# Byshx/Poccala

Hardware: AMD Instinct MI355X
Metric: frames/sec GMM-score+fwd-bwd, 39-d MFCC, 2048-mix (higher is better)
Workload: dtype f32-class (f16x2 split operands, f32 accumulate; f64 dynamic programming)

## Files before the change

poccala_amd/csrc/gmm_score_split.hip:

```cpp
#include <stdlib.h>

#include "pcl_internal.h"

namespace {

#ifndef PCL_SPLIT_WG
#define PCL_SPLIT_WG 256
#endif
constexpr int WG = PCL_SPLIT_WG;
typedef float f16v __attribute__((ext_vector_type(16)));

#ifndef PCL_SPLIT16_NT
#define PCL_SPLIT16_NT 2
#endif
#ifndef PCL_SPLIT16_MINW
#define PCL_SPLIT16_MINW 3
#endif
#ifndef PCL_SPLIT16_MTS
#define PCL_SPLIT16_MTS 1
#endif
typedef _Float16 h8v __attribute__((ext_vector_type(8)));

template <int D, int NT>
__global__ __launch_bounds__(WG, PCL_SPLIT16_MINW * 256 / WG > 0 ? PCL_SPLIT16_MINW * 256 / WG : 1) void gmm_score_split16_kernel(
    const float *__restrict__ frames, const uint4 *__restrict__ pm, const float *__restrict__ fscale, const float *__restrict__ centers,
    int nmt_max, const ScoreTile *__restrict__ tiles, const ScoreSeg *__restrict__ segs, double *__restrict__ out,
    int *__restrict__ flags, const double *__restrict__ kzero, const int *__restrict__ n_on_pipe, const int *__restrict__ npt) {
    static_assert(D % 8 != 0, "the folded constants need a spare slot");
    constexpr int KS8 = (D + 7) / 8;
    constexpr int CH = 2 * KS8;
    constexpr int SC = D / 8, JC = D % 8;
    constexpr float FMAXH = 6.0e4f;
    const ScoreTile tile = tiles[blockIdx.x];
    const int lane = threadIdx.x & 63;
    const int wave = threadIdx.x >> 6;
    const int half = lane >> 5;
    const int col = lane & 31;
    if (tile.seg_lo >= tile.seg_hi) {
        if (threadIdx.x == 0) flags[blockIdx.x] = 0;
        return;
    }
    const int n_mtiles = npt[tile.state];
    __shared__ int s_ovf;
    if (threadIdx.x == 0) s_ovf = 0;
    __syncthreads();
    const int vend = segs[tile.seg_hi - 1].vstart + segs[tile.seg_hi - 1].len;
    const bool wave_active = tile.vstart + wave * NT * 32 < vend;
    if (n_mtiles == 0) {
        if (wave_active) {
            for (int c = 0; c < NT; ++c) {
                const int v = tile.vstart + (wave * NT + c) * 32 + col;
                if (v < vend && half == 0) {
                    int lo = tile.seg0;
                    const int hi = tile.seg_hi - 1;
                    while (lo < hi && segs[lo + 1].vstart <= v) ++lo;
                    const ScoreSeg sg = segs[lo];
                    out[sg.out0 + (long long)(v - sg.vstart) * sg.out_stride] = -INFINITY;
                }
            }
        }
        if (threadIdx.x == 0) flags[blockIdx.x] = 0;
        return;
    }

    h8v xb[NT][2][KS8];
    long long oidx[NT];
    bool valid[NT];
    const float *cen = centers + (size_t)tile.state * D;
    const float *fs = fscale + ((size_t)tile.state * 2 + half) * (KS8 * 8);
    bool ovf = false;
#pragma unroll
    for (int c = 0; c < NT; ++c) {
        int v = tile.vstart + (wave * NT + c) * 32 + col;
        valid[c] = v < vend;
        if (!valid[c]) v = tile.vstart;
        int lo = tile.seg0, hi = tile.seg_hi - 1;
        if (lo < hi && segs[lo + 1].vstart <= v) {
            ++lo;
            if (lo < hi && segs[lo + 1].vstart <= v) {
                ++lo;
                while (lo < hi) {
                    int mid = (lo + hi + 1) >> 1;
                    if (segs[mid].vstart <= v) lo = mid; else hi = mid - 1;
                }
            }
        }
        const ScoreSeg sg = segs[lo];
        const long long t = v - sg.vstart;
        const float *fp = frames + (sg.frame0 + t) * D;
#pragma unroll
        for (int s = 0; s < KS8; ++s)
#pragma unroll
            for (int j = 0; j < 8; ++j) {
                const int d = 8 * s + j;
                float val = 0.f;
                if (d < D) {
                    const float xc = fp[d] - cen[d];
                    val = (half ? xc : xc * xc) * fs[d];
                    ovf |= __builtin_fabsf(val) > FMAXH;
                    val = __builtin_fminf(__builtin_fmaxf(val, -FMAXH), FMAXH);
                }
                if (d == D) val = half ? 0.f : 1.f;
                const _Float16 h1 = (_Float16)val;
                xb[c][0][s][j] = h1;
                xb[c][1][s][j] = (_Float16)(val - (float)h1);
            }
        oidx[c] = sg.out0 + t * (long long)sg.out_stride;
    }
    if (__any(ovf) && lane == 0) s_ovf = 1;

    float sm[NT], ref[NT];
    bool inited[NT];
#pragma unroll
    for (int c = 0; c < NT; ++c) {
        sm[c] = 0.f;
        ref[c] = 0.f;
        inited[c] = false;
    }
    bool ref_ovf = false;

    constexpr int MTS = PCL_SPLIT16_MTS;
    __shared__ __attribute__((aligned(16))) uint4 abuf[2][MTS * CH * 64];
    const uint4 *pstate = pm + (size_t)tile.state * nmt_max * (CH * 64);
    const int wave_s = __builtin_amdgcn_readfirstlane(wave);
    auto dma = [&](int buf, int stage) {
        const uint4 *src = pstate + (size_t)stage * (MTS * CH * 64);
        const int nch = min(MTS, n_mtiles - stage * MTS) * CH;
        if constexpr (KS8 > 5) {
            for (int p = wave; p < nch; p += WG / 64)
                __builtin_amdgcn_global_load_lds((const __attribute__((address_space(1))) void *)(src + p * 64 + lane),
                                                 (__attribute__((address_space(3))) void *)&abuf[buf][p * 64], 16, 0, 0);
            return;
        }
#pragma unroll
        for (int i = 0; i < (MTS * CH + WG / 64 - 1) / (WG / 64); ++i) {
            const int p = wave_s + i * (WG / 64);
            if (p < nch)
                __builtin_amdgcn_global_load_lds((const __attribute__((address_space(1))) void *)(src + p * 64 + lane),
                                                 (__attribute__((address_space(3))) void *)&abuf[buf][p * 64], 16, 0, 0);
        }
    };

#ifdef PCL_SPLIT_STAMPS
    unsigned long long st_acc[4] = {0, 0, 0, 0}, st_t = 0;
#define SSTAMP(k) { const unsigned long long t_ = __builtin_amdgcn_s_memtime(); st_acc[k] += t_ - st_t; st_t = t_; }
#else
#define SSTAMP(k)
#endif
    auto process = [&](int mt) {
        const uint4 *ab = &abuf[(mt / MTS) & 1][(mt % MTS) * (CH * 64)];
        f16v acc[NT];
#pragma unroll
        for (int c = 0; c < NT; ++c)
#pragma unroll
            for (int r = 0; r < 16; ++r) acc[c][r] = 0.f;
        auto frag = [&](int pa, int s) { return *reinterpret_cast<const h8v *>(&ab[(pa * KS8 + s) * 64 + lane]); };
        auto mfma = [&](const h8v &a, int c, int pb, int s) { acc[c] = __builtin_amdgcn_mfma_f32_32x32x16_f16(a, xb[c][pb][s], acc[c], 0, 0, 0); };
        float es[8], eh, snew[NT];
        auto lse_op = [&](int c, int k) {
            if (k < 24) {
                const int r = k / 3;
                if (k % 3 == 0) es[r] = __builtin_amdgcn_exp2f(acc[c][r]);
                else if (k % 3 == 1) eh = __builtin_amdgcn_exp2f(acc[c][r + 8]);
                else es[r] += eh;
            } else if (k < 28) es[k - 24] += es[k - 24 + 4];
            else if (k < 30) es[k - 28] += es[k - 28 + 2];
            else if (k == 30) es[0] += es[1];
            else snew[c] = sm[c] + es[0];
        };
        if constexpr (KS8 <= 5) {
            h8v af[2 * KS8];
            auto rd = [&](int f) { af[f] = frag(f < KS8 ? 1 : 0, f % KS8); };
            constexpr int LATE = KS8 > 2 ? 2 : 0;
            rd(0);
            rd(1);
            __builtin_amdgcn_sched_barrier(0);
#ifdef PCL_SPLIT_PRIO
            __builtin_amdgcn_s_setprio(1);
#endif
#pragma unroll
            for (int s = 0; s < KS8; ++s) {
#pragma unroll
                for (int c = 0; c < NT; ++c) {
                    mfma(af[s], c, 0, s);
                    if (s == 0 && c == 0) {
                        __builtin_amdgcn_sched_barrier(0);
#pragma unroll
                        for (int f = 2; f < 2 * KS8 - LATE; ++f) rd(f);
                    }
                }
                if (s == 2) {
#pragma unroll
                    for (int f = 2 * KS8 - LATE; f < 2 * KS8; ++f) rd(f);
                }
                __builtin_amdgcn_sched_barrier(0);
            }
#pragma unroll
            for (int c = 0; c < NT; ++c) {
                int k = 0;
#pragma unroll
                for (int g = 0; g < 2 * KS8; ++g) {
                    mfma(af[KS8 + g % KS8], c, g < KS8 ? 1 : 0, g % KS8);
                    if (c == 0) __builtin_amdgcn_sched_barrier(0);
#ifndef PCL_DIAG_NOLSE
                    if (c > 0) {
#pragma unroll
                        for (int q = 0; q < 3 && k < 32; ++q, ++k) lse_op(c - 1, k);
                        __builtin_amdgcn_sched_barrier(0);
                    }
#endif
                }
#ifndef PCL_DIAG_NOLSE
                if (c > 0) {
#pragma unroll
                    for (; k < 32; ++k) lse_op(c - 1, k);
                }
#endif
                __builtin_amdgcn_sched_barrier(0);
            }
        } else {
            auto pass = [&](int pa, int pb) {
#pragma unroll
                for (int s = 0; s < KS8; ++s) {
                    const h8v a = frag(pa, s);
#pragma unroll
                    for (int c = 0; c < NT; ++c) mfma(a, c, pb, s);
                }
            };
            pass(1, 0);
            pass(0, 1);
            pass(0, 0);
#ifndef PCL_DIAG_NOLSE
#pragma unroll
            for (int c = 0; c + 1 < NT; ++c)
#pragma unroll
                for (int k = 0; k < 32; ++k) lse_op(c, k);
#endif
        }
#ifndef PCL_DIAG_NOLSE
#pragma unroll
        for (int k = 0; k < 32; ++k) lse_op(NT - 1, k);
#endif
        SSTAMP(1)
#ifdef PCL_SPLIT_PRIO
        __builtin_amdgcn_s_setprio(0);
#endif
#ifdef PCL_DIAG_NOLSE
#pragma unroll
        for (int c = 0; c < NT; ++c) sm[c] += acc[c][0] + acc[c][15];
        return;
#endif
#pragma unroll
        for (int c = 0; c < NT; ++c) {
            if (__any(!inited[c]) | __any(!(snew[c] < 3.0e38f))) {
                float gm = acc[c][0];
#pragma unroll
                for (int r = 1; r < 16; ++r) gm = __builtin_fmaxf(gm, acc[c][r]);
                const float gp = __builtin_fmaxf(gm, __shfl_xor(gm, 32, 64));
                float s = sm[c];
                const bool first = !inited[c];
                if ((first || gp > 0.f) && gp > -5.0e4f) {
                    const _Float16 r1 = (_Float16)__builtin_fminf(__builtin_fmaxf(-(ref[c] + gp), -FMAXH), FMAXH);
                    const float nref = -(float)r1, dl = nref - ref[c];
                    ref_ovf |= __builtin_fabsf(nref) > 5.0e4f;
#ifdef PCL_LSE_FLUSH_REPRO
                    s = first ? 0.f : s * __builtin_amdgcn_exp2f(-dl);
#else
                    const float hs = __builtin_amdgcn_exp2f(-0.5f * dl);
                    s = first ? 0.f : (s * hs) * hs;
#endif
                    inited[c] = true;
#pragma unroll
                    for (int r = 0; r < 16; ++r) acc[c][r] -= dl;
                    ref[c] = nref;
                    if (half) xb[c][0][SC][JC] = r1;
                }
#pragma unroll
                for (int r = 0; r < 16; ++r) s += __builtin_amdgcn_exp2f(acc[c][r]);
                sm[c] = s;
            } else {
                sm[c] = snew[c];
            }
        }
        SSTAMP(2)
    };
    const int n_stages = (n_mtiles + MTS - 1) / MTS;
    dma(0, 0);
#ifdef PCL_SPLIT_STAMPS
    st_t = __builtin_amdgcn_s_memtime();
#endif
    for (int st = 0; st < n_stages; ++st) {
        asm volatile("s_waitcnt vmcnt(0)" ::: "memory");
        SSTAMP(3)
        __syncthreads();
        SSTAMP(0)
        if (st == 0 && threadIdx.x == 0) flags[blockIdx.x] = s_ovf;
        if (st + 1 < n_stages) dma((st + 1) & 1, st + 1);
        if (wave_active) {
            const int mend = min(n_mtiles, (st + 1) * MTS);
            for (int mt = st * MTS; mt < mend; ++mt) process(mt);
        }
    }
#ifdef PCL_SPLIT_STAMPS
    if (blockIdx.x == 800 && lane == 0)
        printf("wave %d: per m-tile: dma-wait %llu  barrier %llu  dma-issue+lds+mfma %llu  lse %llu (memtime ticks)\n", wave,
               st_acc[3] / n_mtiles, st_acc[0] / n_mtiles, st_acc[1] / n_mtiles, st_acc[2] / n_mtiles);
#endif
    constexpr double LN2 = 0.693147180559945309417232121458;
    const double k0 = kzero[tile.state];
    if (wave_active && n_on_pipe[tile.state] > 0) {
#pragma unroll
        for (int c = 0; c < NT; ++c) ref_ovf |= !inited[c];
    }
#pragma unroll
    for (int c = 0; c < NT; ++c) {
        const double S = (double)sm[c] + (double)__shfl_xor(sm[c], 32, 64);
        if (valid[c] && half == 0) out[oidx[c]] = (S > 0) ? LN2 * ((double)ref[c] + k0 + ::log2(S)) : -INFINITY;
    }
    if (__any(ref_ovf) && lane == 0) s_ovf = 1;
    __syncthreads();
    if (threadIdx.x == 0 && s_ovf) flags[blockIdx.x] = 1;
}

template <int D>
void launch16_t(pcl_ctx *ctx, pcl_batch *b, const ScoreTile *tiles, int n_tiles) {
    constexpr size_t static_lds = 2 * (size_t)(2 * ((D + 7) / 8)) * 64 * 16;
    const size_t pad = (ctx->score_wgs_per_cu == 2 && static_lds < (56u << 10)) ? (56u << 10) - static_lds : 0;
    hipLaunchKernelGGL((gmm_score_split16_kernel<D, PCL_SPLIT16_NT>), dim3(n_tiles), dim3(WG), pad, ctx->stream, ctx->frames32,
                       reinterpret_cast<const uint4 *>(ctx->pm16f.p), ctx->fscale, ctx->centers32, ctx->Mpad32 / 32, tiles, b->d_segs,
                       b->Bt, b->d_tile_flags, ctx->kzero, ctx->d_non, ctx->d_npt);
}

}

int pcl_score_split16_tile_frames() { return WG / 64 * PCL_SPLIT16_NT * 32; }

int pcl_launch_score_split16(pcl_ctx *ctx, pcl_batch *b, const ScoreTile *tiles, int n_tiles) {
    if (n_tiles == 0) return PCL_OK;
    pcl_timer_begin(ctx, "score");
    switch (ctx->D) {
#define CASE(DD) case DD: launch16_t<DD>(ctx, b, tiles, n_tiles); break;
        PCL_MFMA_DIMS(CASE)
#undef CASE
        default: PCL_FAIL(ctx, PCL_ERR_INVALID, "internal: no split-f16 scoring kernel for D=%d", ctx->D);
    }
    pcl_timer_end(ctx, "score");
    HIPCHK(ctx, hipGetLastError());
    return PCL_OK;
}
```

Before: 21.64 million.

## Generalize LDS double buffer into configurable ring with partial vmcnt waits

Replaces the fixed two-buffer LDS prefetch of Gaussian parameter tiles with a templated ring of R stages. When R>2 it waits only on older loads via partial vmcnt counts and uses a raw barrier. It also raises the default number of m-tiles per stage from one to two, halving barriers per tile at the cost of more LDS per workgroup. Static asserts check that the ring still fits three workgroups per CU.

```diff
diff --git a/poccala_amd/csrc/gmm_score_split.hip b/poccala_amd/csrc/gmm_score_split.hip
--- a/poccala_amd/csrc/gmm_score_split.hip
+++ b/poccala_amd/csrc/gmm_score_split.hip
@@ -16,10 +16,31 @@
 #ifndef PCL_SPLIT16_MINW
 #define PCL_SPLIT16_MINW 3
 #endif
+#ifndef PCL_SPLIT16_RING
+#define PCL_SPLIT16_RING 2
+#endif
 #ifndef PCL_SPLIT16_MTS
-#define PCL_SPLIT16_MTS 1
+#define PCL_SPLIT16_MTS 2
 #endif
 typedef _Float16 h8v __attribute__((ext_vector_type(8)));
+
+template <int D>
+struct Ring {
+    static constexpr int KS8 = (D + 7) / 8;
+    static constexpr int R = KS8 > 5 ? 2 : PCL_SPLIT16_RING;
+    static constexpr int MTS = KS8 > 5 ? 1 : PCL_SPLIT16_MTS;
+    static constexpr int STAGE_CH = MTS * 2 * KS8;
+    static constexpr size_t LDS = (size_t)R * STAGE_CH * 64 * 16 + 16;
+    static_assert(R >= 2 && MTS >= 1, "a ring has at least two stages");
+    static_assert(3 * LDS <= (160u << 10), "three workgroups per CU: the ring does not fit a third of the 160 KB of LDS");
+    static_assert(LDS <= (56u << 10), "pcl_score_occupancy(ctx, 2) pads a workgroup to 56 KB");
+};
+
+template <int N>
+__device__ __forceinline__ void wait_vmcnt() {
+    static_assert(N >= 0 && N < 64, "vmcnt is a 6-bit counter");
+    asm volatile("s_waitcnt vmcnt(%0)" ::"n"(N) : "memory");
+}
 
 template <int D, int NT>
 __global__ __launch_bounds__(WG, PCL_SPLIT16_MINW * 256 / WG > 0 ? PCL_SPLIT16_MINW * 256 / WG : 1) void gmm_score_split16_kernel(
@@ -119,8 +140,8 @@
     }
     bool ref_ovf = false;
 
-    constexpr int MTS = PCL_SPLIT16_MTS;
-    __shared__ __attribute__((aligned(16))) uint4 abuf[2][MTS * CH * 64];
+    constexpr int R = Ring<D>::R, MTS = Ring<D>::MTS;
+    __shared__ __attribute__((aligned(16))) uint4 abuf[R][MTS * CH * 64];
     const uint4 *pstate = pm + (size_t)tile.state * nmt_max * (CH * 64);
     const int wave_s = __builtin_amdgcn_readfirstlane(wave);
     auto dma = [&](int buf, int stage) {
@@ -135,9 +156,15 @@
 #pragma unroll
         for (int i = 0; i < (MTS * CH + WG / 64 - 1) / (WG / 64); ++i) {
             const int p = wave_s + i * (WG / 64);
-            if (p < nch)
+            if (p >= nch) continue;
+            if constexpr (R == 2) {
                 __builtin_amdgcn_global_load_lds((const __attribute__((address_space(1))) void *)(src + p * 64 + lane),
                                                  (__attribute__((address_space(3))) void *)&abuf[buf][p * 64], 16, 0, 0);
+            } else {
+                const unsigned lds = (unsigned)(size_t)(__attribute__((address_space(3))) char *)&abuf[buf][p * 64];
+                asm volatile("s_mov_b32 m0, %0\n\ts_nop 0\n\tglobal_load_lds_dwordx4 %1, off"
+                             :: "s"(lds), "v"(src + p * 64 + lane) : "memory");
+            }
         }
     };
 
@@ -148,7 +175,7 @@
 #define SSTAMP(k)
 #endif
     auto process = [&](int mt) {
-        const uint4 *ab = &abuf[(mt / MTS) & 1][(mt % MTS) * (CH * 64)];
+        const uint4 *ab = &abuf[(unsigned)(mt / MTS) % R][(mt % MTS) * (CH * 64)];
         f16v acc[NT];
 #pragma unroll
         for (int c = 0; c < NT; ++c)
@@ -286,16 +313,30 @@
     };
     const int n_stages = (n_mtiles + MTS - 1) / MTS;
     dma(0, 0);
+#pragma unroll
+    for (int s = 1; s < R - 1; ++s)
+        if (s < n_stages) dma(s, s);
 #ifdef PCL_SPLIT_STAMPS
     st_t = __builtin_amdgcn_s_memtime();
 #endif
+    constexpr int NW = WG / 64, YLO = (R - 2) * ((MTS * CH) / NW), YHI = (R - 2) * ((MTS * CH) / NW + 1);
     for (int st = 0; st < n_stages; ++st) {
-        asm volatile("s_waitcnt vmcnt(0)" ::: "memory");
+        if (R > 2 && (st + R - 1) * MTS <= n_mtiles) {
+            if (wave_s < (MTS * CH) % NW) wait_vmcnt<YHI>(); else wait_vmcnt<YLO>();
+        } else {
+            wait_vmcnt<0>();
+        }
         SSTAMP(3)
-        __syncthreads();
+        if constexpr (R == 2) {
+            __syncthreads();
+        } else {
+            asm volatile("s_waitcnt lgkmcnt(0)" ::: "memory");
+            __builtin_amdgcn_s_barrier();
+            asm volatile("" ::: "memory");
+        }
         SSTAMP(0)
         if (st == 0 && threadIdx.x == 0) flags[blockIdx.x] = s_ovf;
-        if (st + 1 < n_stages) dma((st + 1) & 1, st + 1);
+        if (st + R - 1 < n_stages) dma((unsigned)(st + R - 1) % R, st + R - 1);
         if (wave_active) {
             const int mend = min(n_mtiles, (st + 1) * MTS);
             for (int mt = st * MTS; mt < mend; ++mt) process(mt);
@@ -324,7 +365,7 @@
 
 template <int D>
 void launch16_t(pcl_ctx *ctx, pcl_batch *b, const ScoreTile *tiles, int n_tiles) {
-    constexpr size_t static_lds = 2 * (size_t)(2 * ((D + 7) / 8)) * 64 * 16;
+    constexpr size_t static_lds = Ring<D>::LDS;
     const size_t pad = (ctx->score_wgs_per_cu == 2 && static_lds < (56u << 10)) ? (56u << 10) - static_lds : 0;
     hipLaunchKernelGGL((gmm_score_split16_kernel<D, PCL_SPLIT16_NT>), dim3(n_tiles), dim3(WG), pad, ctx->stream, ctx->frames32,
                        reinterpret_cast<const uint4 *>(ctx->pm16f.p), ctx->fscale, ctx->centers32, ctx->Mpad32 / 32, tiles, b->d_segs,
```

After: 22.37 million (median of 6 runs). 1.03x the previous value.
